# fdrmrc/Polydeal

Hardware: AMD Instinct MI355X
Metric: assembled DoF/s (SIP Poisson, p=3, 3D) (higher is better)
Workload: dtype f64

## Files before the change

### polydeal_amd/csrc/host/polydeal_host.h

```cpp
#pragma once

#include "../../../include/polydeal_hip.h"
#include "../pdh_basis.h"

#include <algorithm>
#include <array>
#include <cmath>
#include <cstdint>
#include <cstdlib>
#include <cstring>
#include <exception>
#include <fstream>
#include <map>
#include <mutex>
#include <thread>
#include <random>
#include <stdexcept>
#include <string>
#include <unordered_map>
#include <utility>
#include <vector>

namespace polydeal_hip
{
constexpr int invalid_index = -1;

inline void qgauss_1d_compute(int n, std::vector<double> &x, std::vector<double> &w)
{
  x.assign(n, 0.0);
  w.assign(n, 0.0);
  const long double pi = 3.14159265358979323846264338327950288L;
  for (int i = 0; i < n; ++i)
    {
      long double t = -std::cos(pi * (i + 0.75L) / (n + 0.5L));
      long double dp = 1.0L;
      for (int it = 0; it < 100; ++it)
        {
          long double p0 = 1.0L, p1 = t;
          for (int k = 1; k < n; ++k)
            {
              const long double p2 = ((2 * k + 1) * t * p1 - k * p0) / (k + 1);
              p0 = p1;
              p1 = p2;
            }
          dp = n * (p0 - t * p1) / (1 - t * t);
          const long double dt = p1 / dp;
          t -= dt;
          if (std::fabs((double)dt) < 1e-19)
            break;
        }
      {
        long double p0 = 1.0L, p1 = t;
        for (int k = 1; k < n; ++k)
          {
            const long double p2 = ((2 * k + 1) * t * p1 - k * p0) / (k + 1);
            p0 = p1;
// ... 493 lines not shown
      xi[ax] = side;
      if (dim == 2)
        {
          const int qq = rev ? nqf - 1 - q : q;
          xi[tang[0]] = x1[qq];
          w = w1[qq];
        }
      else
        {
          xi[tang[0]] = x1[q % nqf];
          xi[tang[1]] = x1[q / nqf];
          w = w1[q % nqf] * w1[q / nqf];
        }
      q1_map(g, cell, xi, x, J);
      double nr[3] = {0, 0, 0}, area;
      if (dim == 2)
        {
          const double t0 = J[0][tang[0]], t1 = J[1][tang[0]];
          area = std::sqrt(t0 * t0 + t1 * t1);
          nr[0] = t1;
          nr[1] = -t0;
        }
      else
        {
          const double a[3] = {J[0][tang[0]], J[1][tang[0]], J[2][tang[0]]};
          const double b[3] = {J[0][tang[1]], J[1][tang[1]], J[2][tang[1]]};
          nr[0] = a[1] * b[2] - a[2] * b[1];
          nr[1] = a[2] * b[0] - a[0] * b[2];
          nr[2] = a[0] * b[1] - a[1] * b[0];
          area = std::sqrt(nr[0] * nr[0] + nr[1] * nr[1] + nr[2] * nr[2]);
        }
      double nn = 0.0, dot = 0.0;
      for (int c = 0; c < dim; ++c)
        nn += nr[c] * nr[c];
      nn = std::sqrt(nn);
      for (int c = 0; c < dim; ++c)
        {
          nr[c] /= nn;
          dot += nr[c] * J[c][ax] * (side ? 1.0 : -1.0);
        }
      const double sgn = dot < 0 ? -1.0 : 1.0;
      for (int c = 0; c < dim; ++c)
        {
          out.x.push_back(x[c]);
          out.n.push_back(sgn * nr[c]);
        }
      out.w.push_back(w * area);
    }
}

template <class F>
inline void parallel_for(size_t n, F &&fn)
{
  unsigned nt = std::thread::hardware_concurrency();
  if (const char *e = std::getenv("PDH_HOST_THREADS"))
    nt = (unsigned)std::max(1, std::atoi(e));
  nt = std::max(1u, std::min<unsigned>(nt, 64u));
  if (nt == 1 || n < 256)
    {
      for (size_t i = 0; i < n; ++i)
        fn(i);
      return;
    }
  std::vector<std::thread> th;
  std::exception_ptr err;
  std::mutex mx;
  const size_t chunk = (n + nt - 1) / nt;
  for (unsigned t = 0; t < nt; ++t)
    {
      const size_t b = (size_t)t * chunk, e = std::min(n, b + chunk);
      if (b >= e)
        break;
      th.emplace_back([&, b, e] {
        try
          {
            for (size_t i = b; i < e; ++i)
              fn(i);
          }
        catch (...)
          {
            std::lock_guard<std::mutex> lk(mx);
            err = std::current_exception();
          }
      });
    }
  for (auto &t : th)
    t.join();
  if (err)
    std::rethrow_exception(err);
}

inline void cell_quadrature_soa(const BackgroundGrid &g, int cell, int nq, const double *x1, const double *w1, double *X,
                                size_t stride, size_t at, double *W)
{
  const int dim = g.dim;
  const int np = (dim == 2) ? nq * nq : nq * nq * nq;
  for (int q = 0; q < np; ++q)
    {
      const int i[3] = {q % nq, (q / nq) % nq, q / (nq * nq)};
      double xi[3], x[3], J[3][3], w = 1.0;
      for (int c = 0; c < dim; ++c)
        {
          xi[c] = x1[i[c]];
          w *= w1[i[c]];
        }
      q1_map(g, cell, xi, x, J);
      double det;
      if (dim == 2)
        det = J[0][0] * J[1][1] - J[0][1] * J[1][0];
      else
// ... 1121 lines not shown
```

### polydeal_amd/csrc/pdh_capi.cpp

```cpp
#include "pdh_basis.h"
#include "pdh_combos.h"
#include "pdh_ctx.h"
#include "pdh_kernels.h"
#include "pdh_moment_tables.h"

#include <hip/hip_runtime.h>

#include <algorithm>
#include <chrono>
#include <cmath>
#include <cstdio>
#include <cstdlib>
#include <cstring>
#include <memory>
#include <string>
#include <vector>

static pdh_resolve_fn g_resolve[PDH_N_GROUPS] = {pdh_resolve_g0, pdh_resolve_g1, pdh_resolve_g2, pdh_resolve_g3,
                                                 pdh_resolve_g4, pdh_resolve_g5, pdh_resolve_g6, pdh_resolve_g7};

template <int NT, int LB>
static constexpr int sched_instr(bool sym)
{
  int c = 0;
  for (int a = 0; a < NT; ++a)
    for (int b = 0; b < NT; ++b)
      for (int r = 0; r < 4; ++r)
        if ((sym ? pdh::Sched<NT, LB>::sym_mask(a, b, r) : pdh::Sched<NT, LB>::full_mask(a, b, r)) != 0u)
          ++c;
  return c;
}
static int sched_instr_rt(int nt, int lb, bool sym)
{
  switch (nt * 4 + (lb - 1))
    {
#define PDH_C(NT, LB)                                                                              \
  case NT * 4 + (LB - 1):                                                                          \
    return sched_instr<NT, LB>(sym);
      PDH_C(1, 1) PDH_C(1, 2) PDH_C(1, 3) PDH_C(1, 4) PDH_C(2, 1) PDH_C(2, 2) PDH_C(2, 3) PDH_C(2, 4)
      PDH_C(3, 1) PDH_C(3, 2) PDH_C(3, 3) PDH_C(3, 4) PDH_C(4, 1) PDH_C(4, 2) PDH_C(4, 3) PDH_C(4, 4)
#undef PDH_C
    }
  return 0;
}

static void free_problem(pdh_ctx *ctx)
{
  for (void *p : ctx->prob.allocs)
    (void)hipFree(p);
  ctx->prob.drop_graph();
  ctx->prob = pdh_ctx::Problem{};
}

#ifndef PDH_SRC_HASH
#define PDH_SRC_HASH "unhashed"
#endif
extern "C" const char *pdh_version(void) { return "polydeal_hip 0.4+" PDH_SRC_HASH " gfx950"; }

extern "C" const char *pdh_last_error(const pdh_ctx *ctx) { return ctx ? ctx->err.c_str() : pdh_noctx_error().c_str(); }

extern "C" int pdh_create(pdh_ctx **out, int device_id)
{
  if (!out)
    return fail(nullptr, PDH_EINVAL, "pdh_create: out is NULL");
  *out = nullptr;
  int ndev = 0;
  hipError_t e = hipGetDeviceCount(&ndev);
  if (e != hipSuccess || ndev <= 0)
    return fail(nullptr, PDH_EDEVICE,
                std::string("pdh_create: no HIP device available (") + hipGetErrorString(e) +
                  "); this library has no CPU fallback");
  if (device_id < 0 || device_id >= ndev)
    return fail(nullptr, PDH_EINVAL, "pdh_create: device_id out of range");
  PDH_HIP(nullptr, hipSetDevice(device_id));
  pdh_ctx *ctx = new pdh_ctx;
  ctx->device = device_id;
  if (hipStreamCreateWithFlags(&ctx->stream2, hipStreamNonBlocking) != hipSuccess ||
      hipEventCreateWithFlags(&ctx->ev_fork, hipEventDisableTiming) != hipSuccess ||
      hipEventCreateWithFlags(&ctx->ev_join, hipEventDisableTiming) != hipSuccess)
    {
      delete ctx;
      return fail(nullptr, PDH_EDEVICE, "pdh_create: second stream / events");
    }
  if (hipStreamCreate(&ctx->own_stream) != hipSuccess)
    {
      delete ctx;
      return fail(nullptr, PDH_EDEVICE, "pdh_create: hipStreamCreate failed");
    }
  ctx->stream = ctx->own_stream;
  *out = ctx;
  return PDH_OK;
}

extern "C" void pdh_destroy(pdh_ctx *ctx)
{
  if (!ctx)
    return;
  (void)hipSetDevice(ctx->device);
  (void)hipStreamSynchronize(ctx->stream);
  pdh_mg_detach(ctx);
  free_problem(ctx);
  for (DevBuf *b : {&ctx->io.in0, &ctx->io.in1, &ctx->io.ptr, &ctx->io.out, &ctx->io.grad, &ctx->io.err, &ctx->shape_midx, &ctx->checksum})
    b->release();
  if (ctx->pinned)
    (void)hipHostFree(ctx->pinned);
  for (auto &ev : ctx->events)
    if (ev)
      (void)hipEventDestroy(ev);
  (void)hipStreamDestroy(ctx->own_stream);
  if (ctx->stream2)
    (void)hipStreamDestroy(ctx->stream2);
  if (ctx->ev_fork)
    (void)hipEventDestroy(ctx->ev_fork);
  if (ctx->ev_join)
    (void)hipEventDestroy(ctx->ev_join);
  delete ctx;
}

extern "C" int pdh_terms_merge_stats(pdh_ctx *ctx, int64_t *out4)
{
  if (!ctx || !out4)
    return fail(ctx, PDH_EINVAL, "ctx and out4 are required");
  if (!ctx->prob.resident)
    return fail(ctx, PDH_ESTATE, "pdh_terms_merge_stats called before pdh_set_problem");
  for (int i = 0; i < 4; ++i)
    out4[i] = ctx->prob.row_kernel == RowKernel::terms ? ctx->prob.terms_merge[i] : 0;
  return PDH_OK;
}

struct GaussRule01
{
  double x[PDH_MAX_N1D] = {0}, w[PDH_MAX_N1D] = {0};
  explicit GaussRule01(int n)
  {
    std::vector<long double> gx, gw;
    pdh::gauss_legendre01(n, gx, gw);
    for (int i = 0; i < n; ++i)
      x[i] = (double)gx[i], w[i] = (double)gw[i];
  }
};

static int pack_faces_on_device(pdh_ctx *ctx, const pdh_problem *p, const Packed &K, PdhDev &D)
{
  const int dim = p->dim;
  const int64_t nap = K.n_ap, nqf = K.nqf_src, nruns = (int64_t)K.pk_at.size();
  double *out[5] = {nullptr, nullptr, nullptr, nullptr, nullptr};
  const size_t out_n[5] = {(size_t)dim * nap, (size_t)dim * nap, (size_t)nap, (size_t)nap, (size_t)nap};
  for (int k = 0; k < 5; ++k)
    PDH_TRY(device_buffer(ctx, out_n[k], &out[k], "packed face points"));
  D.ap_x = out[0], D.ap_n = out[1], D.ap_wself = out[2], D.ap_wcross = out[3], D.ap_sig = out[4];
  if (nruns == 0 || nap == 0)
    return PDH_OK;
// ... 155 lines not shown
  ctx->prob.face_runs.reserve(K.run_ap.size());
  for (size_t r = 0; r < K.run_ap.size(); ++r)
    ctx->prob.face_runs.push_back({K.run_ap[r], K.run_fq[r], K.run_cnt[r], K.run_bdry[r], K.run_slot[r]});
  ctx->prob.n_rows_owned = (int64_t)K.n_owned * K.n;
  ctx->prob.n_rows_total = p->n_rows;
  ctx->prob.max_row_len = K.max_row_len;
  ctx->prob.h_blk_ptr = K.blk_ptr;
  ctx->prob.h_blk_dof = K.blk_dof;
  ctx->prob.h_slot_dof.resize((size_t)K.n_owned);
  for (int s = 0; s < K.n_owned; ++s)
    ctx->prob.h_slot_dof[(size_t)s] = p->dof_offset[K.own_agg[(size_t)s]];
  ctx->prob.n_agg_total = p->n_agg;
  const int64_t i_sym = sched_instr_rt(K.NT, K.LB, true), i_full = sched_instr_rt(K.NT, K.LB, false);
  const int ch_d = (K.NT >= 3) ? 64 : 32, ch_o = 32;
  auto ksteps = [](int64_t npts, int ch) {
    int64_t s = (npts / ch) * (ch / 4);
    const int64_t rem = npts % ch;
    return s + (rem + 3) / 4;
  };
  int64_t kv = 0, kf = 0, ko = 0;
  for (size_t sl = 0; sl < K.own_agg.size(); ++sl)
    {
      kv += ksteps(K.vq_ptr[sl + 1] - K.vq_ptr[sl], ch_d);
      kf += ksteps(K.ap_ptr[sl + 1] - K.ap_ptr[sl], ch_d);
    }
  for (size_t it = 0; it < K.it_pcnt.size(); ++it)
    ko += ksteps(K.it_pcnt[it], ch_o);
  ctx->prob.mfma_diag = kv * (p->dim + (p->reaction_c != 0.0 ? 1 : 0)) * i_sym + kf * 2 * i_sym;
  ctx->prob.mfma_offdiag = ko * 2 * i_full;
  if (K.tiled)
    {
      const int64_t nt = (K.n + 63) / 64, i64 = sched_instr_rt(4, 4, true);
      ctx->prob.mfma_diag = (kv * (p->dim + (p->reaction_c != 0.0 ? 1 : 0)) + kf * 2) * (64 * (nt * (nt - 1) / 2) + i64 * nt);
      ctx->prob.mfma_offdiag = ko * 2 * 64 * nt * nt;
    }
}

static int upload_rows_state(pdh_ctx *ctx, const Packed &K, const KernelPlan &plan, int cus)
{
  const RowsHost &RH = plan.rows;
  PdhRows &R = ctx->prob.rows;
  PDH_UP(RH.fr_ptr, R.fr_ptr);
  PDH_UP(RH.fr_pbeg, R.fr_pbeg);
  PDH_UP(RH.fr_pcnt, R.fr_pcnt);
  PDH_UP(RH.fr_nbr, R.fr_nbr);
  PDH_UP(RH.fr_axis, R.fr_axis);
  PDH_UP(RH.fr_blk, R.fr_blk);
  PDH_UP(RH.fr_flags, R.fr_flags);
  PDH_UP(RH.fr_coord, R.fr_coord);
  PDH_UP(RH.fr_sigma, R.fr_sigma);
  PDH_UP(RH.fr_nsign, R.fr_nsign);
  PDH_UP(RH.meta, R.meta);
  PDH_TRY(device_buffer(ctx, 16, &R.sched, "row kernel: work counter"));
  PDH_HIP(ctx, hipMemset(R.sched, 0, 16 * sizeof(unsigned int)));
  const size_t n_stamps = (size_t)std::max(K.n_owned, 1) * 16;
  PDH_TRY(device_buffer(ctx, n_stamps, &R.stamps, "row kernel: stamps"));
  PDH_HIP(ctx, hipMemset(R.stamps, 0, n_stamps * sizeof(long long)));
  if (RH.multi)
    {
      const int waves = cus * 8;
      const size_t stride = std::max<size_t>((size_t)RH.maxf * 64, (size_t)RH.maxs * 32 + 64);
      PDH_TRY(device_buffer(ctx, (size_t)waves * stride, &R.m2c_scratch, "row kernel: MULTI scratch"));
      R.scratch_waves = waves;
      R.scratch_stride = (int64_t)stride;
    }
  R.tensor_only = plan.tensor_only ? 1 : 0;
  R.multi = RH.multi ? 1 : 0;
  R.maxe = RH.maxe;
  R.maxf = RH.maxf;
  R.vq_tensor_n = plan.vq_n;
  R.fq_tensor_n = RH.fq_tensor_n;
  return PDH_OK;
}

static int upload_terms_state(pdh_ctx *ctx, const Packed &K, const KernelPlan &plan)
{
  const TermsHost &TH = plan.terms;
  PdhTerms &T = ctx->prob.terms;
  PDH_UP(TH.meta, T.meta);
  PDH_UP(TH.sf_pt, T.sf_pt);
  PDH_UP(TH.sf_info, T.sf_info);
  PDH_UP(TH.sf_ivl, T.sf_ivl);
  PDH_UP(TH.cell_ivl, T.cell_ivl);
  T.maxruns = TH.maxruns, T.maxsf = TH.maxsf, T.maxsi = TH.maxsi, T.maxcell = TH.maxcell;
  T.vq_tensor_n = plan.vq_n, T.fq_tensor_n = plan.rows.fq_tensor_n;
  T.lds_bytes = TH.lds_bytes;
  T.split = TH.split;
  T.task_pts = TH.task_pts;
  T.tpm = TH.task_pts > 4 ? 8 : 4;
  T.tstride = pdht::terms_task_doubles(T.maxsf, T.maxcell, T.tpm);
  const size_t n_tdata = (size_t)std::max(K.n_owned, 1) * T.tstride;
  double *tdata = nullptr;
  PDH_TRY(device_buffer(ctx, n_tdata, &tdata, "term kernel: records of 1-D rules"));
  PDH_HIP(ctx, hipMemsetAsync(tdata, 0, n_tdata * sizeof(double), ctx->stream));
  T.tdata = tdata;
  PDH_HIP(ctx, pdh_launch_terms_gather(&ctx->prob.dev, &T, tdata, K.n_owned, ctx->stream));
  PDH_HIP(ctx, hipStreamSynchronize(ctx->stream));
  const size_t n_stamps = (size_t)std::max(K.n_owned, 1) * 16;
  PDH_TRY(device_buffer(ctx, n_stamps, &T.stamps, "term kernel: stamps"));
  PDH_HIP(ctx, hipMemset(T.stamps, 0, n_stamps * sizeof(long long)));
  PDH_TRY(device_buffer(ctx, 16, &T.sched, "term kernel: work counter"));
  PDH_HIP(ctx, hipMemset(T.sched, 0, 16 * sizeof(unsigned int)));
  ctx->prob.terms_merge[0] = TH.n_cells_in, ctx->prob.terms_merge[1] = TH.n_cells_out;
  ctx->prob.terms_merge[2] = TH.n_sf_in, ctx->prob.terms_merge[3] = TH.n_sf_out;
  return PDH_OK;
}

static void resolve_launches(pdh_ctx *ctx, const Packed &K, const PlanSwitches &sw, int cus, const char **why_row)
{
  *why_row = nullptr;
  pdh_ctx::Problem &pr = ctx->prob;
  const PdhDev &D = pr.dev;
  const bool reaction = D.reaction_c != 0.0;
  if (K.tiled)
    pdh_resolve_tiled(D.dim, D.n1d, D.n, reaction, pr.n_diag_slots, pr.n_items, pr.direct);
  else
    g_resolve[combo_group(D.dim, D.n1d, K.NT, K.LB)](D.dim, D.n1d, K.NT, K.LB, reaction, pr.n_diag_slots, pr.n_items, pr.direct);
  if (pr.d_mtab)
    pdh_resolve_moment(D.n1d, D.n, pr.n_diag_slots, pr.n_items, pr.moment);
  if (pr.row_kernel == RowKernel::rows)
    pr.row = pdh_resolve_rows(&D, &pr.rows, pr.n_owned, cus, sw.rows_waves_per_cu, sw.rows_lds_pad, sw.rows_verbose, &pr.row_zero_sched);
  else if (pr.row_kernel == RowKernel::terms)
    {
      const char *why = nullptr;
      pr.row = pdh_resolve_terms(&D, &pr.terms, pr.n_owned, cus, sw.terms_wg_waves, sw.terms_wg_batch, pdht::WG_STORE_AUX,
                                 pdht::WG_DRAIN ? 1 : 0, &why);
      if (!pr.row.kernel)
        *why_row = why;
    }
}

static int set_problem_impl(pdh_ctx *ctx, const pdh_problem *p, int32_t row_begin, int32_t row_end, const pdh_cartesian_points *cart);

extern "C" int pdh_set_problem_local(pdh_ctx *ctx, const pdh_problem *p, int32_t row_begin, int32_t row_end)
{
  return set_problem_impl(ctx, p, row_begin, row_end, nullptr);
}

extern "C" int pdh_set_problem_cartesian(pdh_ctx *ctx, const pdh_problem *p, const pdh_cartesian_points *points, int32_t row_begin,
                                         int32_t row_end)
{
  if (!points)
    return fail(ctx, PDH_EINVAL, "points is NULL");
  return set_problem_impl(ctx, p, row_begin, row_end, points);
}

static int set_problem_impl(pdh_ctx *ctx, const pdh_problem *p, int32_t row_begin, int32_t row_end, const pdh_cartesian_points *cart)
{
  PDH_TRY(need_ctx(ctx));
  if (cart && ctx->exchange_mode == PDH_EXCHANGE_GHOST)
    return fail(ctx, PDH_EUNSUPPORTED, "the cartesian description runs owner-computes-rows only (no ghost-block exchange)");
  PDH_HIP(ctx, hipSetDevice(ctx->device));
  PDH_HIP(ctx, hipStreamSynchronize(ctx->stream));
  free_problem(ctx);
  ++ctx->values_gen;
  ++ctx->problem_epoch;
  struct FreeUnlessDone
  {
    pdh_ctx *ctx;
    bool done = false;
    ~FreeUnlessDone()
    {
      if (!done)
        free_problem(ctx);
    }
  } guard{ctx};
  const PlanSwitches sw = read_plan_switches();
  auto t_last = std::chrono::steady_clock::now();
  auto lap = [&](const char *what) {
    if (!sw.trace)
      return;
    const auto now = std::chrono::steady_clock::now();
    fprintf(stderr, "[pdh_set_problem] %-32s %7.1f ms\n", what, std::chrono::duration<double, std::milli>(now - t_last).count());
    t_last = now;
  };
  lap("wait for the stream, free the old problem");

  std::unique_ptr<Packed> K_owner(new Packed);
  Packed &K = *K_owner;
  PDH_TRY(pack_problem(ctx->err, p, row_begin, row_end, K, ctx->exchange_mode, cart));
  lap("validate + repack (host)");
  auto plan = std::make_unique<KernelPlan>(plan_kernels(p, K, sw));
  lap("row kernel plan (host)");
  if (cart && plan->kernel != RowKernel::terms)
    return fail(ctx, PDH_EUNSUPPORTED, "cartesian description: the term kernels do not apply (a polytope's tables exceed their LDS budget, "
                                       "or the element has none): describe the problem with its points (pdh_set_problem)");
  PDH_TRY(upload_problem(ctx, p, K));
  record_problem(ctx, p, K);
  lap("upload: state of every kernel");
  int cus = 256;
  (void)hipDeviceGetAttribute(&cus, hipDeviceAttributeMultiprocessorCount, ctx->device);
  if (plan->kernel == RowKernel::rows)
    {
      PDH_TRY(upload_rows_state(ctx, K, *plan, cus));
      lap("upload: pdh_rows.h state");
    }
  else if (plan->kernel == RowKernel::terms)
    {
      PDH_TRY(upload_terms_state(ctx, K, *plan));
      lap("upload: term kernel state");
    }
  ctx->prob.row_kernel = plan->kernel;
  ctx->prob.why_terms = plan->why_terms;
  const char *why_row = nullptr;
  resolve_launches(ctx, K, sw, cus, &why_row);
  if (why_row)
    return fail(ctx, PDH_EUNSUPPORTED, std::string("the row kernel chosen for this problem cannot be launched on this device: ") + why_row);
  ctx->prob.resident = true;
  ctx->ev_used = 0;
  guard.done = true;
  K_owner.reset();
  plan.reset();
  lap("release host staging");
  return PDH_OK;
}

extern "C" int pdh_set_algorithm(pdh_ctx *ctx, int algorithm)
{
  PDH_TRY(need_ctx(ctx));
  if (algorithm != PDH_ALG_AUTO && algorithm != PDH_ALG_DIRECT && algorithm != PDH_ALG_MOMENT && algorithm != PDH_ALG_ROWS)
    return fail(ctx, PDH_EINVAL, "algorithm must be PDH_ALG_AUTO, PDH_ALG_DIRECT, PDH_ALG_MOMENT or PDH_ALG_ROWS");
  ctx->algorithm = algorithm;
  return PDH_OK;
}

extern "C" int pdh_algorithm_in_use(pdh_ctx *ctx)
{
  if (!resident(ctx))
    return fail(ctx, PDH_ESTATE, "no problem resident");
  if (ctx->use_rows())
    return PDH_ALG_ROWS;
  const bool d = ctx->use_moment(0), o = ctx->use_moment(1);
  return d && o ? PDH_ALG_MOMENT : (d || o ? PDH_ALG_MIXED : PDH_ALG_DIRECT);
}

extern "C" int pdh_rows_kernel_in_use(pdh_ctx *ctx)
{
  if (!resident(ctx))
    return fail(ctx, PDH_ESTATE, "no problem resident");
  if (!ctx->use_rows())
    return PDH_ROWS_NONE;
  if (ctx->prob.row_kernel == RowKernel::terms)
    return PDH_ROWS_TERMS;
  if (ctx->prob.rows.multi)
    return PDH_ROWS_MULTI;
  return ctx->prob.dev.n == 64 ? PDH_ROWS_PIECES : PDH_ROWS_STREAMED;
}

extern "C" int pdh_set_problem(pdh_ctx *ctx, const pdh_problem *p)
{
  if (!p)
    return fail(ctx, PDH_EINVAL, "problem is NULL");
  return pdh_set_problem_local(ctx, p, 0, p->n_rows);
}

static int take_events(pdh_ctx *ctx, hipEvent_t (&e)[4])
{
  for (hipEvent_t &x : e)
    x = ctx->next_event();
  if (!e[0] || !e[1] || !e[2] || !e[3])
    return fail(ctx, PDH_EDEVICE, "hipEventCreate failed");
  return PDH_OK;
}

extern "C" int pdh_assemble_device(pdh_ctx *ctx)
{
// ... 144 lines not shown
    return fail(ctx, PDH_EINVAL, "n_ranks is smaller than the number of ranks in agg_rank, or an output is NULL");
  for (int r = 0; r < n_ranks; ++r)
    {
      send_count[r] = r < (int)ctx->prob.send_count.size() ? ctx->prob.send_count[r] : 0;
      recv_count[r] = r < (int)ctx->prob.recv_count.size() ? ctx->prob.recv_count[r] : 0;
    }
  return PDH_OK;
}

extern "C" int pdh_exchange_get_send(pdh_ctx *ctx, double *d_send)
{
  if (!resident(ctx) || !ctx->prob.ghost)
    return fail(ctx, PDH_ESTATE, "no problem resident in PDH_EXCHANGE_GHOST mode");
  if (ctx->prob.n_send == 0)
    return PDH_OK;
  if (!d_send)
    return fail(ctx, PDH_EINVAL, "d_send is NULL");
  PDH_HIP(ctx, hipSetDevice(ctx->device));
  PDH_HIP(ctx, hipMemcpyAsync(d_send, ctx->prob.dev.values + ctx->prob.n_values, ctx->prob.n_send * sizeof(double), hipMemcpyDeviceToDevice,
                              ctx->stream));
  return PDH_OK;
}

extern "C" int pdh_exchange_apply(pdh_ctx *ctx, const double *d_recv)
{
  if (!resident(ctx) || !ctx->prob.ghost)
    return fail(ctx, PDH_ESTATE, "no problem resident in PDH_EXCHANGE_GHOST mode");
  ++ctx->values_gen;
  if (ctx->prob.n_recv == 0)
    return PDH_OK;
  if (!d_recv)
    return fail(ctx, PDH_EINVAL, "d_recv is NULL");
  PDH_HIP(ctx, hipSetDevice(ctx->device));
  PDH_HIP(ctx, pdh_launch_ghost_apply(&ctx->prob.dev, d_recv, ctx->prob.n_r21, ctx->prob.d_r21_src, ctx->prob.d_r21_dst, ctx->prob.d_r21_rlen, ctx->prob.n_r22,
                                      ctx->prob.d_r22_ptr, ctx->prob.d_r22_src, ctx->prob.d_r22_slot, ctx->stream));
  return PDH_OK;
}

extern "C" int pdh_set_stream(pdh_ctx *ctx, void *stream)
{
  PDH_TRY(need_ctx(ctx));
  PDH_HIP(ctx, hipSetDevice(ctx->device));
  PDH_HIP(ctx, hipStreamSynchronize(ctx->stream));
  ctx->stream = stream ? (hipStream_t)stream : ctx->own_stream;
  return PDH_OK;
}

extern "C" int pdh_debug_rows_stamps(pdh_ctx *ctx, long long *out)
{
  const long long *src = !ctx || !ctx->prob.resident ? nullptr
                         : ctx->prob.row_kernel == RowKernel::terms ? ctx->prob.terms.stamps
                         : ctx->prob.row_kernel == RowKernel::rows ? ctx->prob.rows.stamps
                                                                : nullptr;
  if (!src || !out)
    return fail(ctx, PDH_ESTATE, "no row-kernel problem resident");
  PDH_HIP(ctx, hipSetDevice(ctx->device));
  PDH_HIP(ctx, hipStreamSynchronize(ctx->stream));
  PDH_HIP(ctx, hipMemcpy(out, src, (size_t)ctx->prob.n_owned * 16 * sizeof(long long), hipMemcpyDeviceToHost));
  return PDH_OK;
}

#ifdef PDHT_VARIANTS
extern "C" int pdh_debug_terms_wg_variant(pdh_ctx *ctx, int order, int aux, int drain)
{
  if (!ctx || !ctx->prob.resident || ctx->prob.row_kernel != RowKernel::terms || ctx->prob.dev.n1d != 4 || ctx->prob.dev.n != 64)
    return fail(ctx, PDH_ESTATE, "no FE_DGQ(3) term-kernel problem resident");
  if (order != 0)
    return fail(ctx, PDH_EINVAL, "order must be 0 (piece-major)");
  PDH_HIP(ctx, hipSetDevice(ctx->device));
  PDH_HIP(ctx, hipStreamSynchronize(ctx->stream));
  const PlanSwitches sw = read_plan_switches();
  int cus = 256;
  (void)hipDeviceGetAttribute(&cus, hipDeviceAttributeMultiprocessorCount, ctx->device);
  const char *why = nullptr;
  const PdhLaunch L = pdh_resolve_terms(&ctx->prob.dev, &ctx->prob.terms, ctx->prob.n_owned, cus, sw.terms_wg_waves, sw.terms_wg_batch, aux,
                                        drain, &why);
  if (!L.kernel)
    return fail(ctx, PDH_EUNSUPPORTED, why);
  ctx->prob.row = L;
  return PDH_OK;
}
#endif

extern "C" int pdh_set_overlap(pdh_ctx *ctx, int enabled)
{
  PDH_TRY(need_ctx(ctx));
  ctx->overlap = enabled != 0;
  return PDH_OK;
}

extern "C" int pdh_synchronize(pdh_ctx *ctx)
{
  PDH_TRY(need_ctx(ctx));
  PDH_HIP(ctx, hipSetDevice(ctx->device));
  PDH_HIP(ctx, hipStreamSynchronize(ctx->stream));
  return PDH_OK;
}

extern "C" void *pdh_stream(pdh_ctx *ctx) { return ctx ? (void *)ctx->stream : nullptr; }

extern "C" int pdh_assemble(pdh_ctx *ctx, double *values)
{
  if (!values)
    return fail(ctx, PDH_EINVAL, "values is NULL");
  int rc = pdh_assemble_device(ctx);
  if (rc != PDH_OK)
// ... 121 lines not shown
```

### polydeal_amd/csrc/pdh_ctx.h

```cpp
#pragma once
#include "../../include/polydeal_hip.h"
#include "pdh_launch.h"
#include "pdh_plan.h"

#include <hip/hip_runtime.h>

#include <algorithm>
#include <cstdint>
#include <memory>
#include <string>
#include <utility>
#include <vector>

class DevBuf
{
public:
  enum Policy { exact, slack };
  DevBuf() = default;
  explicit DevBuf(Policy p) : policy(p) {}
  DevBuf(const DevBuf &) = delete;
  DevBuf &operator=(const DevBuf &) = delete;
  DevBuf &operator=(DevBuf &&o) noexcept
  {
    release();
    std::swap(p, o.p);
    std::swap(bytes, o.bytes);
    return *this;
  }
  ~DevBuf() { release(); }
  void release()
  {
    if (p)
      (void)hipFree(p);
    p = nullptr;
    bytes = 0;
  }
  template <class T>
  T *get(size_t count)
  {
    const size_t need = std::max<size_t>(count, 1) * sizeof(T);
    if (need > bytes)
      {
        release();
        const size_t want = policy == slack ? need + need / 4 + 256 : need;
        if (hipMalloc(&p, want) != hipSuccess)
          {
            p = nullptr;
            return nullptr;
          }
        bytes = want;
      }
    return static_cast<T *>(p);
  }
  template <class T>
  T *ptr() const
  {
    return static_cast<T *>(p);
  }

private:
  Policy policy = exact;
  void *p = nullptr;
  size_t bytes = 0;
};

struct pdh_ctx
{
  int device = 0;
  hipStream_t stream = nullptr, own_stream = nullptr;
  std::string err;
  hipStream_t stream2 = nullptr;
  hipEvent_t ev_fork = nullptr, ev_join = nullptr;
  int overlap = 1;
  int algorithm = PDH_ALG_AUTO;
  int exchange_mode = PDH_EXCHANGE_NONE;
  bool profiling = false;
  std::vector<hipEvent_t> events;
  size_t ev_used = 0;
  uint64_t values_gen = 0, prec_gen = 0;
  uint64_t problem_epoch = 0;
  int prec_kind = PDH_PREC_NONE;
  bool prec_ok = true;
  uint64_t prec_epoch = 0;
  struct pdh_mg *mg = nullptr;
  bool mg_gone = false;
  struct Io
  {
    DevBuf in0{DevBuf::slack}, in1{DevBuf::slack}, ptr{DevBuf::slack}, out{DevBuf::slack}, grad{DevBuf::slack}, err{DevBuf::slack};
  } io;
  int shape_key = -1;
  DevBuf shape_midx;
  DevBuf checksum;
  double *pinned = nullptr;

  struct Problem
  {
    bool resident = false;
    std::vector<void *> allocs;
    PdhDev dev{};
    int n_owned = 0, n_items = 0, NT = 0;
    bool tiled = false;
    PdhLaunch direct[3] = {}, moment[2] = {}, row = {};
    bool row_zero_sched = false;
    int64_t terms_merge[4] = {0, 0, 0, 0};
    int64_t n_values = 0, n_vq = 0, n_ap = 0;
    int64_t mfma_diag = 0, mfma_offdiag = 0;
    int basis = 0;
    const double *d_mtab = nullptr;
    int64_t n_rows_owned = 0, n_rows_total = 0;
    int32_t n_agg_total = 0;
    struct FaceRun { int64_t ap_begin, fq_begin; int32_t count; int32_t boundary; int32_t slot; };
    std::vector<FaceRun> face_runs;
    const int64_t *d_vq_src = nullptr, *d_ap_src = nullptr, *d_bd_rng = nullptr;
    int64_t n_vq_caller = 0, n_fq_caller = 0;
    std::vector<int32_t> cart_fq_face;
    int cart_nqf = 0;
    bool ghost = false;
    int n_diag_slots = 0, n_r21 = 0, n_r22 = 0;
    int64_t n_send = 0, n_recv = 0;
    std::vector<int64_t> send_count, recv_count;
    const int64_t *d_r21_src = nullptr, *d_r21_dst = nullptr, *d_r22_ptr = nullptr, *d_r22_src = nullptr;
    const int32_t *d_r21_rlen = nullptr, *d_r22_slot = nullptr;
    RowKernel row_kernel = RowKernel::none;
    PdhRows rows{};
    PdhTerms terms{};
    hipGraphExec_t graph_exec = nullptr;
    int graph_state = 0, graph_alg = -1;
    hipStream_t graph_stream = nullptr;
    void drop_graph()
    {
      if (graph_exec)
        (void)hipGraphExecDestroy(graph_exec);
      graph_exec = nullptr;
// ... 191 lines not shown
```

### polydeal_amd/csrc/pdh_plan.cpp

```cpp
#include "pdh_plan_internal.h"

#include "pdh_basis.h"
#include "pdh_combos.h"
#include "pdh_rows_tables.h"
#include "pdh_terms_tables.h"

#include <chrono>
#include <cstdio>

static thread_local std::string g_err_noctx;
std::string &pdh_noctx_error() { return g_err_noctx; }

int combo_group(int dim, int n1d, int nt, int lb)
{
#define PDH_X(G, D, N, T, L)                                                                       \
  if (dim == D && n1d == N && nt == T && lb == L)                                                  \
    return G;
  PDH_COMBOS(PDH_X)
#undef PDH_X
  return -1;
}


namespace
// ... 1356 lines not shown
    }
  T.task_pts = std::max(vq_n * ivl_c, fn * ivl_f);
  tlap("maxima");
  {
    const int one = pdht::terms_lds_bytes(K.n1d, basis, T.maxruns, T.maxsf, T.maxsi, T.maxcell, 0);
    const int two = pdht::terms_lds_bytes(K.n1d, basis, T.maxruns, T.maxsf, T.maxsi, T.maxcell, 1);
    auto waves = [](int bytes) { return bytes <= 0 ? 0 : std::min(12, (int)(160 * 1024 / (((int64_t)bytes + 1279) / 1280 * 1280))); };
    T.split = sw.terms_split >= 0 ? sw.terms_split : ((waves(two) > waves(one) && K.n <= 20) ? 1 : 0);
    if (pdht::terms_has_kind(K.n1d, basis) == 2)
      T.split = 0;
    T.lds_bytes = T.split ? two : one;
  }
  if (T.lds_bytes <= 0 || T.lds_bytes > PDH_TERMS_LDS_CAP)
    return refuse(why, "term kernel: the tables of the largest polytope do not fit its LDS budget (moment-based kinds take over)");
  T.maxsf = std::max(T.maxsf, 1);
  T.maxcell = std::max(T.maxcell, 1);
  T.sf_pt.assign((size_t)K.n_owned * T.maxsf, 0);
  T.sf_info.assign((size_t)K.n_owned * T.maxsf, 0);
  T.sf_ivl.assign((size_t)K.n_owned * T.maxsf * 2 * TERMS_MI, 0);
  T.cell_ivl.assign((size_t)K.n_owned * T.maxcell * 3 * TERMS_MI, -1);
  T.meta.assign((size_t)K.n_owned * (pdht::TERMS_HDR + T.maxruns * pdht::TERMS_ENT), 0.0);
  const bool ok = host_parallel_all((size_t)K.n_owned, [&](size_t sl) { return write_terms_of_slot(p, K, A.order[sl], MG[sl], sl, T); });
  tlap("tables");
  return ok || refuse(why, "term kernel: run order");
}

PlanSwitches read_plan_switches()
{
  PlanSwitches s;
  auto first = [](const char *name) { return getenv(name) ? getenv(name)[0] : '\0'; };
  s.terms_merge = first("PDH_TERMS_MERGE") == '0' ? 0 : (first("PDH_TERMS_MERGE") == '2' ? 2 : 1);
  s.terms_split = getenv("PDH_TERMS_SPLIT") ? (first("PDH_TERMS_SPLIT") == '1' ? 1 : 0) : -1;
  s.trace = getenv("PDH_TRACE_SETUP") != nullptr;
  s.rows_verbose = getenv("PDH_ROWS_VERBOSE") != nullptr;
  s.terms_off = first("PDH_TERMS") == '0';
  s.terms_dgq3_off = first("PDH_TERMS_DGQ3") == '0';
  s.rows_waves_per_cu = getenv("PDH_ROWS_WAVES_PER_CU") ? atoi(getenv("PDH_ROWS_WAVES_PER_CU")) : 0;
  s.rows_lds_pad = getenv("PDH_ROWS_LDS_PAD") ? (size_t)atol(getenv("PDH_ROWS_LDS_PAD")) : 0;
  s.terms_wg_waves = getenv("PDH_TERMS_WG_WAVES") && atoi(getenv("PDH_TERMS_WG_WAVES")) == 4 ? 4 : 8;
  s.terms_wg_batch = getenv("PDH_TERMS_WG_BATCH") ? atoi(getenv("PDH_TERMS_WG_BATCH")) : 0;
  return s;
}

KernelPlan plan_kernels(const pdh_problem *p, const Packed &K, const PlanSwitches &sw)
{
  KernelPlan P;
  RowsHost &RH = P.rows;
  FaceAnalysis A;
  if (p->dim != 3 || K.n1d < 2 || K.n1d > 4 || K.ghost)
    {
      P.why_rows = P.why_terms = K.ghost ? "exchange variant" : "not 3-D FE_DGQ / FE_AggloDGP of degree 1 .. 3";
      return P;
    }
  if (K.cart)
    {
      RH.planar_ok = true;
      RH.fq_tensor_n = K.cart->nqf;
      RH.fast_j.assign(3 * K.run_ap.size(), 0);
      order_runs_of_slots(K, A);
      P.vq_n = K.cart->nq;
      P.why_rows = "cartesian description: the kinds of pdh_rows.h need the points";
    }
  else if (analyse_faces(p, K, RH, A, &P.why_rows) && build_rows_tables(p, K, A, sw, RH, &P.why_rows) &&
           rows_kind_applies(p, K, RH, P.vq_n, P.tensor_only, &P.why_rows))
    P.kernel = RowKernel::rows;
  const int terms_kind = pdht::terms_has_kind(K.n1d, p->basis == PDH_BASIS_AGGLODGP ? 1 : 0);
  if (!RH.planar_ok)
    P.why_terms = P.why_rows;
  else if (!K.cart && (sw.terms_off || (terms_kind == 2 && sw.terms_dgq3_off)))
    P.why_terms = "term kernel: switched off (PDH_TERMS / PDH_TERMS_DGQ3)";
  else
    {
      if (P.vq_n < 0 && RH.fq_tensor_n > 0)
        P.vq_n = resolve_volume_rules(p, K);
      if (build_terms_tables(p, K, RH, A, std::max(P.vq_n, 0), sw, P.terms, &P.why_terms))
        P.kernel = RowKernel::terms;
    }
  return P;
}

static int check_plan(const pdh_problem *p, int32_t row_begin, int32_t row_end, KernelPlan &plan)
{
  Packed K;
  g_err_noctx.clear();
  PDH_TRY(pack_problem(g_err_noctx, p, row_begin, row_end, K));
  PlanSwitches sw = read_plan_switches();
  sw.terms_off = sw.terms_dgq3_off = false;
  plan = plan_kernels(p, K, sw);
  return PDH_OK;
}

extern "C" int pdh_check_rows(const pdh_problem *p, int32_t row_begin, int32_t row_end)
{
  KernelPlan plan;
  PDH_TRY(check_plan(p, row_begin, row_end, plan));
  if (plan.kernel != RowKernel::none)
    return 1;
  g_err_noctx = plan.why_rows;
  if (plan.rows.planar_ok && plan.rows.fq_tensor_n > 0 && plan.vq_n > 0)
    g_err_noctx += "; " + plan.why_terms;
  return 0;
}

extern "C" int pdh_check_terms(const pdh_problem *p, int32_t row_begin, int32_t row_end, int64_t *stats5)
{
  KernelPlan plan;
  PDH_TRY(check_plan(p, row_begin, row_end, plan));
  const TermsHost &TH = plan.terms;
  if (stats5 && plan.rows.planar_ok)
    {
      stats5[0] = TH.maxruns, stats5[1] = TH.maxsf, stats5[2] = TH.maxsi, stats5[3] = TH.maxcell, stats5[4] = TH.lds_bytes;
    }
  if (plan.kernel == RowKernel::terms)
    return 1;
  g_err_noctx = plan.why_terms;
  return 0;
}

extern "C" int pdh_check_problem(const pdh_problem *p, int32_t row_begin, int32_t row_end, int64_t *stats)
{
  Packed K;
  g_err_noctx.clear();
  const int rc = pack_problem(g_err_noctx, p, row_begin, row_end, K);
  if (rc == PDH_OK && stats)
    {
      stats[0] = (int64_t)K.n_owned;
      stats[1] = (int64_t)K.it_own.size();
      stats[2] = K.n_vq;
      stats[3] = K.n_ap;
// ... 119 lines not shown
```

### polydeal_amd/csrc/pdh_plan.h

```cpp
#pragma once
#include "../../include/polydeal_hip.h"
#include "pdh_dev.h"

#include <algorithm>
#include <cstdint>
#include <cstdlib>
#include <memory>
#include <string>
#include <thread>
#include <vector>

template <class F>
void host_parallel_for(size_t n, F &&fn)
{
  unsigned nt = std::thread::hardware_concurrency();
  if (const char *e = std::getenv("PDH_HOST_THREADS"))
    nt = (unsigned)std::max(1, std::atoi(e));
  nt = std::max(1u, std::min<unsigned>(nt, 64u));
  if (nt == 1 || n < 256)
    {
      for (size_t i = 0; i < n; ++i)
        fn(i);
      return;
    }
  std::vector<std::thread> th;
  const size_t chunk = (n + nt - 1) / nt;
  for (unsigned t = 0; t < nt; ++t)
    {
      const size_t b = (size_t)t * chunk, e = std::min(n, b + chunk);
      if (b >= e)
        break;
      th.emplace_back([&fn, b, e] {
        for (size_t i = b; i < e; ++i)
          fn(i);
      });
    }
  for (auto &t : th)
    t.join();
}

enum class RowKernel { none, rows, terms };

template <class T>
struct UninitAlloc : std::allocator<T>
{
  template <class U>
  struct rebind { using other = UninitAlloc<U>; };
  template <class U, class... A>
  void construct(U *ptr, A &&...a)
  {
    if constexpr (sizeof...(A) == 0)
      ::new ((void *)ptr) U;
    else
      ::new ((void *)ptr) U(std::forward<A>(a)...);
  }
};
using dvec = std::vector<double, UninitAlloc<double>>;

struct Packed
{
  int n = 0, n1d = 0, NT = 0, LB = 0;
  bool tiled = false;
  std::vector<int32_t> midx;
  PdhBasisTab tab;
  std::vector<int32_t> own_agg, own_row, row_len, diag_L, it_own, it_nbr, it_pcnt, it_pos, it_nbr_slot, it_pos_t;
  std::vector<int64_t> row_base, vq_ptr, ap_ptr, it_pbeg;
  std::vector<int64_t> blk_ptr{0};
  std::vector<int32_t> blk_dof;
  int max_row_len = 0;
  dvec vq_x, vq_w;
  std::vector<int64_t> pk_at, pk_fq;
// ... 24 lines not shown
    const int64_t i = pk_fq[r] + q;
    return (pk_flags[r] & 2) ? 0.0 : (src->fq_w_out ? src->fq_w_out[i] : src->fq_w[i]);
  }
  int64_t n_values = 0;
  int n_owned = 0;
  std::vector<int64_t> send_count, recv_count;
  int64_t n_send = 0, n_recv = 0;
  std::vector<int32_t> r21_rlen, r22_slot;
  std::vector<int64_t> r21_src, r21_dst, r22_ptr, r22_src;
};

struct RowsHost
{
  std::vector<int32_t> fr_ptr, fr_pcnt, fr_nbr, fr_axis, fr_blk, fr_flags;
  std::vector<int64_t> fr_pbeg;
  std::vector<double> fr_coord, fr_sigma, fr_nsign;
  std::vector<double> meta;
  int fq_tensor_n = 0;
  bool multi = false;
  int maxe = 16, maxf = 6;
  int maxs = 0;
  bool planar_ok = false;
  std::vector<signed char> fast_j;
};

struct TermsHost
{
  std::vector<double> meta;
  std::vector<int64_t> sf_pt;
  std::vector<int32_t> sf_info, sf_ivl, cell_ivl;
  int maxruns = 0, maxsf = 0, maxsi = 0, maxcell = 0, lds_bytes = 0, split = 0, task_pts = 0;
  int64_t n_cells_in = 0, n_cells_out = 0, n_sf_in = 0, n_sf_out = 0;
};

struct KernelPlan
{
  RowKernel kernel = RowKernel::none;
  RowsHost rows;
  TermsHost terms;
  int vq_n = -1;
  bool tensor_only = false;
  std::string why_rows, why_terms;
};

int pack_problem(std::string &err, const pdh_problem *p, int32_t row_begin, int32_t row_end, Packed &K,
                 int exchange_mode = PDH_EXCHANGE_NONE, const pdh_cartesian_points *cart = nullptr);

struct PlanSwitches
{
  int terms_merge = 1, terms_split = -1;
  bool trace = false, rows_verbose = false, terms_off = false, terms_dgq3_off = false;
  int rows_waves_per_cu = 0, terms_wg_waves = 8, terms_wg_batch = 0;
  size_t rows_lds_pad = 0;
};
PlanSwitches read_plan_switches();

KernelPlan plan_kernels(const pdh_problem *p, const Packed &K, const PlanSwitches &sw);

int combo_group(int dim, int n1d, int nt, int lb);

std::string &pdh_noctx_error();

void pdh_lanczos_tridiagonal(const std::vector<double> &alpha, const std::vector<double> &beta, std::vector<double> &diag,
                             std::vector<double> &offdiag);
void pdh_chebyshev_coefficients(int degree, double estimate, double smoothing_range, double *lambda_lo, double *lambda_hi,
                                std::vector<double> &c1, std::vector<double> &c2);
```

Baseline: 1.670 billion.

## Overlap kernel planning with upload, skip unused plans, and defer host staging release

Runs plan_kernels on an async worker while the problem data uploads, and short-circuits planning to the term kernel when it applies, so the rows tables are never built. It frees host staging buffers on a background thread, makes the stamp buffers compile-time optional, and turns the blocking memsets into async ones. Host thread counts now respect affinity, cgroup quotas and OMP_NUM_THREADS. The target is set-up cost, which only matters if the metric counts assembly set-up. The trade-offs are extra threads competing for CPUs and stamp readout failing in default builds.

After: 1.670 billion, median of 2. Within noise of the previous version (-0.0%).

```diff
diff --git a/polydeal_amd/csrc/host/polydeal_host.h b/polydeal_amd/csrc/host/polydeal_host.h
--- a/polydeal_amd/csrc/host/polydeal_host.h
+++ b/polydeal_amd/csrc/host/polydeal_host.h
@@ -2,6 +2,7 @@
 
 #include "../../../include/polydeal_hip.h"
 #include "../pdh_basis.h"
+#include "../pdh_host_threads.h"
 
 #include <algorithm>
 #include <array>
@@ -601,10 +602,7 @@
 template <class F>
 inline void parallel_for(size_t n, F &&fn)
 {
-  unsigned nt = std::thread::hardware_concurrency();
-  if (const char *e = std::getenv("PDH_HOST_THREADS"))
-    nt = (unsigned)std::max(1, std::atoi(e));
-  nt = std::max(1u, std::min<unsigned>(nt, 64u));
+  const unsigned nt = pdh_host::loop_threads();
   if (nt == 1 || n < 256)
     {
       for (size_t i = 0; i < n; ++i)
diff --git a/polydeal_amd/csrc/pdh_capi.cpp b/polydeal_amd/csrc/pdh_capi.cpp
--- a/polydeal_amd/csrc/pdh_capi.cpp
+++ b/polydeal_amd/csrc/pdh_capi.cpp
@@ -12,6 +12,7 @@
 #include <cstdio>
 #include <cstdlib>
 #include <cstring>
+#include <future>
 #include <memory>
 #include <string>
 #include <vector>
@@ -98,6 +99,8 @@
     return;
   (void)hipSetDevice(ctx->device);
   (void)hipStreamSynchronize(ctx->stream);
+  if (ctx->host_release.valid())
+    ctx->host_release.wait();
   pdh_mg_detach(ctx);
   free_problem(ctx);
   for (DevBuf *b : {&ctx->io.in0, &ctx->io.in1, &ctx->io.ptr, &ctx->io.out, &ctx->io.grad, &ctx->io.err, &ctx->shape_midx, &ctx->checksum})
@@ -359,10 +362,14 @@
   PDH_UP(RH.fr_nsign, R.fr_nsign);
   PDH_UP(RH.meta, R.meta);
   PDH_TRY(device_buffer(ctx, 16, &R.sched, "row kernel: work counter"));
-  PDH_HIP(ctx, hipMemset(R.sched, 0, 16 * sizeof(unsigned int)));
+  PDH_HIP(ctx, hipMemsetAsync(R.sched, 0, 16 * sizeof(unsigned int), ctx->stream));
+  R.stamps = nullptr;
+#if defined(PDHR_STAMP) || defined(PDHR_CHECK)
   const size_t n_stamps = (size_t)std::max(K.n_owned, 1) * 16;
   PDH_TRY(device_buffer(ctx, n_stamps, &R.stamps, "row kernel: stamps"));
-  PDH_HIP(ctx, hipMemset(R.stamps, 0, n_stamps * sizeof(long long)));
+  PDH_HIP(ctx, hipMemsetAsync(R.stamps, 0, n_stamps * sizeof(long long), ctx->stream));
+#endif
+  PDH_HIP(ctx, hipStreamSynchronize(ctx->stream));
   if (RH.multi)
     {
       const int waves = cus * 8;
@@ -402,12 +409,15 @@
   PDH_HIP(ctx, hipMemsetAsync(tdata, 0, n_tdata * sizeof(double), ctx->stream));
   T.tdata = tdata;
   PDH_HIP(ctx, pdh_launch_terms_gather(&ctx->prob.dev, &T, tdata, K.n_owned, ctx->stream));
-  PDH_HIP(ctx, hipStreamSynchronize(ctx->stream));
+  T.stamps = nullptr;
+#ifdef PDHT_STAMP
   const size_t n_stamps = (size_t)std::max(K.n_owned, 1) * 16;
   PDH_TRY(device_buffer(ctx, n_stamps, &T.stamps, "term kernel: stamps"));
-  PDH_HIP(ctx, hipMemset(T.stamps, 0, n_stamps * sizeof(long long)));
+  PDH_HIP(ctx, hipMemsetAsync(T.stamps, 0, n_stamps * sizeof(long long), ctx->stream));
+#endif
   PDH_TRY(device_buffer(ctx, 16, &T.sched, "term kernel: work counter"));
-  PDH_HIP(ctx, hipMemset(T.sched, 0, 16 * sizeof(unsigned int)));
+  PDH_HIP(ctx, hipMemsetAsync(T.sched, 0, 16 * sizeof(unsigned int), ctx->stream));
+  PDH_HIP(ctx, hipStreamSynchronize(ctx->stream));
   ctx->prob.terms_merge[0] = TH.n_cells_in, ctx->prob.terms_merge[1] = TH.n_cells_out;
   ctx->prob.terms_merge[2] = TH.n_sf_in, ctx->prob.terms_merge[3] = TH.n_sf_out;
   return PDH_OK;
@@ -459,6 +469,8 @@
     return fail(ctx, PDH_EUNSUPPORTED, "the cartesian description runs owner-computes-rows only (no ghost-block exchange)");
   PDH_HIP(ctx, hipSetDevice(ctx->device));
   PDH_HIP(ctx, hipStreamSynchronize(ctx->stream));
+  if (ctx->host_release.valid())
+    ctx->host_release.wait();
   free_problem(ctx);
   ++ctx->values_gen;
   ++ctx->problem_epoch;
@@ -487,14 +499,35 @@
   Packed &K = *K_owner;
   PDH_TRY(pack_problem(ctx->err, p, row_begin, row_end, K, ctx->exchange_mode, cart));
   lap("validate + repack (host)");
-  auto plan = std::make_unique<KernelPlan>(plan_kernels(p, K, sw));
-  lap("row kernel plan (host)");
+  PlanSwitches sw_plan = sw;
+  sw_plan.only_chosen = true;
+  double plan_ms = 0.0;
+  std::future<KernelPlan> planning = std::async(std::launch::async, [p, &K, sw_plan, &plan_ms] {
+    pdh_host::reserved_cpus() = 1;
+    const auto t0 = std::chrono::steady_clock::now();
+    KernelPlan made = plan_kernels(p, K, sw_plan);
+    plan_ms = std::chrono::duration<double, std::milli>(std::chrono::steady_clock::now() - t0).count();
+    return made;
+  });
+  struct JoinOnExit
+  {
+    std::future<KernelPlan> &f;
+    ~JoinOnExit()
+    {
+      if (f.valid())
+        f.wait();
+    }
+  } join_guard{planning};
+  PDH_TRY(upload_problem(ctx, p, K));
+  record_problem(ctx, p, K);
+  lap("upload: state of every kernel");
+  auto plan = std::make_unique<KernelPlan>(planning.get());
+  if (sw.trace)
+    fprintf(stderr, "[pdh_set_problem] %-32s %7.1f ms (on a worker, beside the upload)\n", "row kernel plan (host)", plan_ms);
+  lap("wait for the plan");
   if (cart && plan->kernel != RowKernel::terms)
     return fail(ctx, PDH_EUNSUPPORTED, "cartesian description: the term kernels do not apply (a polytope's tables exceed their LDS budget, "
                                        "or the element has none): describe the problem with its points (pdh_set_problem)");
-  PDH_TRY(upload_problem(ctx, p, K));
-  record_problem(ctx, p, K);
-  lap("upload: state of every kernel");
   int cus = 256;
   (void)hipDeviceGetAttribute(&cus, hipDeviceAttributeMultiprocessorCount, ctx->device);
   if (plan->kernel == RowKernel::rows)
@@ -516,9 +549,11 @@
   ctx->prob.resident = true;
   ctx->ev_used = 0;
   guard.done = true;
-  K_owner.reset();
-  plan.reset();
-  lap("release host staging");
+  ctx->host_release = std::async(std::launch::async, [k = std::move(K_owner), pl = std::move(plan)]() mutable {
+    pl.reset();
+    k.reset();
+  });
+  lap("hand the host staging to a worker");
   return PDH_OK;
 }
 
@@ -769,6 +804,8 @@
                          : ctx->prob.row_kernel == RowKernel::terms ? ctx->prob.terms.stamps
                          : ctx->prob.row_kernel == RowKernel::rows ? ctx->prob.rows.stamps
                                                                 : nullptr;
+  if (!src && resident(ctx) && ctx->prob.row_kernel != RowKernel::none)
+    return fail(ctx, PDH_ESTATE, "this build of the library writes no stamps (-DPDHR_STAMP / -DPDHT_STAMP)");
   if (!src || !out)
     return fail(ctx, PDH_ESTATE, "no row-kernel problem resident");
   PDH_HIP(ctx, hipSetDevice(ctx->device));
diff --git a/polydeal_amd/csrc/pdh_ctx.h b/polydeal_amd/csrc/pdh_ctx.h
--- a/polydeal_amd/csrc/pdh_ctx.h
+++ b/polydeal_amd/csrc/pdh_ctx.h
@@ -7,6 +7,7 @@
 
 #include <algorithm>
 #include <cstdint>
+#include <future>
 #include <memory>
 #include <string>
 #include <utility>
@@ -79,6 +80,7 @@
   size_t ev_used = 0;
   uint64_t values_gen = 0, prec_gen = 0;
   uint64_t problem_epoch = 0;
+  std::future<void> host_release;
   int prec_kind = PDH_PREC_NONE;
   bool prec_ok = true;
   uint64_t prec_epoch = 0;
diff --git a/polydeal_amd/csrc/pdh_host_threads.h b/polydeal_amd/csrc/pdh_host_threads.h
--- /dev/null
+++ b/polydeal_amd/csrc/pdh_host_threads.h
@@ -0,0 +1,66 @@
+#pragma once
+#include <algorithm>
+#include <cstdio>
+#include <cstdlib>
+#include <thread>
+#if defined(__linux__)
+#include <sched.h>
+#endif
+
+namespace pdh_host
+{
+inline unsigned usable_cpus()
+{
+  static const unsigned found = [] {
+    unsigned n = std::max(1u, std::thread::hardware_concurrency());
+#if defined(__linux__)
+    cpu_set_t set;
+    CPU_ZERO(&set);
+    if (sched_getaffinity(0, sizeof(set), &set) == 0 && CPU_COUNT(&set) > 0)
+      n = std::min(n, (unsigned)CPU_COUNT(&set));
+    auto quota = [&](double q, double period) {
+      if (q > 0 && period > 0)
+        n = std::min(n, (unsigned)std::max(1.0, (q + period - 1) / period));
+    };
+    if (FILE *f = std::fopen("/sys/fs/cgroup/cpu.max", "r"))
+      {
+        double q = 0, period = 0;
+        if (std::fscanf(f, "%lf %lf", &q, &period) == 2)
+          quota(q, period);
+        std::fclose(f);
+      }
+    else
+      {
+        double q = 0, period = 0;
+        FILE *fq = std::fopen("/sys/fs/cgroup/cpu/cpu.cfs_quota_us", "r"), *fp = std::fopen("/sys/fs/cgroup/cpu/cpu.cfs_period_us", "r");
+        if (fq && fp && std::fscanf(fq, "%lf", &q) == 1 && std::fscanf(fp, "%lf", &period) == 1)
+          quota(q, period);
+        if (fq)
+          std::fclose(fq);
+        if (fp)
+          std::fclose(fp);
+      }
+#endif
+    if (const char *e = std::getenv("OMP_NUM_THREADS"))
+      if (std::atoi(e) > 0)
+        n = std::min(n, (unsigned)std::atoi(e));
+    return std::max(1u, std::min(n, 64u));
+  }();
+  return found;
+}
+
+inline unsigned &reserved_cpus()
+{
+  static thread_local unsigned reserved = 0;
+  return reserved;
+}
+
+inline unsigned loop_threads()
+{
+  unsigned nt = usable_cpus();
+  nt = nt > reserved_cpus() ? nt - reserved_cpus() : 1;
+  if (const char *e = std::getenv("PDH_HOST_THREADS"))
+    nt = (unsigned)std::max(1, std::atoi(e));
+  return std::max(1u, std::min<unsigned>(nt, 64u));
+}
+}
diff --git a/polydeal_amd/csrc/pdh_plan.cpp b/polydeal_amd/csrc/pdh_plan.cpp
--- a/polydeal_amd/csrc/pdh_plan.cpp
+++ b/polydeal_amd/csrc/pdh_plan.cpp
@@ -1432,6 +1432,16 @@
       P.why_rows = P.why_terms = K.ghost ? "exchange variant" : "not 3-D FE_DGQ / FE_AggloDGP of degree 1 .. 3";
       return P;
     }
+  auto t_prev = std::chrono::steady_clock::now();
+  auto tlap = [&](const char *what) {
+    const auto now = std::chrono::steady_clock::now();
+    if (sw.trace)
+      fprintf(stderr, "[plan_kernels] %-35s %6.1f ms\n", what, std::chrono::duration<double, std::milli>(now - t_prev).count());
+    t_prev = now;
+  };
+  const int terms_kind = pdht::terms_has_kind(K.n1d, p->basis == PDH_BASIS_AGGLODGP ? 1 : 0);
+  const bool terms_switched_off = !K.cart && (sw.terms_off || (terms_kind == 2 && sw.terms_dgq3_off));
+  bool terms_tried = false;
   if (K.cart)
     {
       RH.planar_ok = true;
@@ -1441,20 +1451,53 @@
       P.vq_n = K.cart->nq;
       P.why_rows = "cartesian description: the kinds of pdh_rows.h need the points";
     }
-  else if (analyse_faces(p, K, RH, A, &P.why_rows) && build_rows_tables(p, K, A, sw, RH, &P.why_rows) &&
-           rows_kind_applies(p, K, RH, P.vq_n, P.tensor_only, &P.why_rows))
-    P.kernel = RowKernel::rows;
-  const int terms_kind = pdht::terms_has_kind(K.n1d, p->basis == PDH_BASIS_AGGLODGP ? 1 : 0);
-  if (!RH.planar_ok)
+  else
+    {
+      const bool faces_ok = analyse_faces(p, K, RH, A, &P.why_rows);
+      tlap("analyse_faces");
+      if (sw.only_chosen && faces_ok && terms_kind != 0 && !terms_switched_off && RH.fq_tensor_n > 0)
+        {
+          P.vq_n = resolve_volume_rules(p, K);
+          tlap("volume rules");
+          terms_tried = true;
+          const bool ok = build_terms_tables(p, K, RH, A, std::max(P.vq_n, 0), sw, P.terms, &P.why_terms);
+          tlap("term tables");
+          if (ok)
+            {
+              P.kernel = RowKernel::terms;
+              P.why_rows = "the kinds of pdh_rows.h were not planned: the term kernels take the problem";
+              return P;
+            }
+        }
+      if (faces_ok)
+        {
+          bool ok = build_rows_tables(p, K, A, sw, RH, &P.why_rows);
+          tlap("rows tables");
+          if (ok)
+            {
+              ok = rows_kind_applies(p, K, RH, P.vq_n, P.tensor_only, &P.why_rows);
+              tlap("rows kinds (volume rules)");
+            }
+          if (ok)
+            P.kernel = RowKernel::rows;
+        }
+    }
+  if (terms_tried)
+    ;
+  else if (!RH.planar_ok)
     P.why_terms = P.why_rows;
-  else if (!K.cart && (sw.terms_off || (terms_kind == 2 && sw.terms_dgq3_off)))
+  else if (terms_switched_off)
     P.why_terms = "term kernel: switched off (PDH_TERMS / PDH_TERMS_DGQ3)";
   else
     {
       if (P.vq_n < 0 && RH.fq_tensor_n > 0)
-        P.vq_n = resolve_volume_rules(p, K);
+        {
+          P.vq_n = resolve_volume_rules(p, K);
+          tlap("volume rules");
+        }
       if (build_terms_tables(p, K, RH, A, std::max(P.vq_n, 0), sw, P.terms, &P.why_terms))
         P.kernel = RowKernel::terms;
+      tlap("term tables");
     }
   return P;
 }
diff --git a/polydeal_amd/csrc/pdh_plan.h b/polydeal_amd/csrc/pdh_plan.h
--- a/polydeal_amd/csrc/pdh_plan.h
+++ b/polydeal_amd/csrc/pdh_plan.h
@@ -1,6 +1,7 @@
 #pragma once
 #include "../../include/polydeal_hip.h"
 #include "pdh_dev.h"
+#include "pdh_host_threads.h"
 
 #include <algorithm>
 #include <cstdint>
@@ -13,10 +14,7 @@
 template <class F>
 void host_parallel_for(size_t n, F &&fn)
 {
-  unsigned nt = std::thread::hardware_concurrency();
-  if (const char *e = std::getenv("PDH_HOST_THREADS"))
-    nt = (unsigned)std::max(1, std::atoi(e));
-  nt = std::max(1u, std::min<unsigned>(nt, 64u));
+  const unsigned nt = pdh_host::loop_threads();
   if (nt == 1 || n < 256)
     {
       for (size_t i = 0; i < n; ++i)
@@ -147,6 +145,7 @@
   bool trace = false, rows_verbose = false, terms_off = false, terms_dgq3_off = false;
   int rows_waves_per_cu = 0, terms_wg_waves = 8, terms_wg_batch = 0;
   size_t rows_lds_pad = 0;
+  bool only_chosen = false;
 };
 PlanSwitches read_plan_switches();
 
```
